# GATB/leon

Hardware: AMD Instinct MI355X
Metric: compressed input MB/s (DNA encode path) (higher is better)
Workload: dtype u64

## Files before the change

leon_amd/capi.py:

```python
import ctypes as C
import os

import numpy as np

_HERE = os.path.dirname(os.path.abspath(__file__))

ABI_VERSION = 5
HEADER_TEXT_DEVICE_CAP = 4096
LEON_F_KEEP_TRACE = 1
LEON_F_DICT_ON_DEVICE = 2


class LeonDnaError(RuntimeError):
    def __init__(self, code, msg):
        super().__init__("leon_dna error %d: %s" % (code, msg))
        self.code = code


def lib_path():
    return os.path.join(_HERE, "lib", "libleon_dna.so")


class _Cfg(C.Structure):
    _fields_ = [("struct_size", C.c_uint32), ("kmer_size", C.c_uint32), ("reads_per_block", C.c_uint32),
# ... 100 lines not shown
    "leon_device_count": (C.c_int, [C.POINTER(C.c_int)]),
    "leon_device_alloc": (C.c_int, [C.c_int, C.c_uint64, C.POINTER(C.c_void_p)]),
    "leon_device_upload": (C.c_int, [C.c_int, C.c_void_p, C.c_void_p, C.c_uint64]),
    "leon_device_copy": (C.c_int, [C.c_int, C.c_void_p, C.c_void_p, C.c_uint64]),
    "leon_device_download": (C.c_int, [C.c_int, C.c_void_p, C.c_void_p, C.c_uint64]),
    "leon_host_qual_encode_blocks": (C.c_int, [C.c_char_p, _u64p, C.c_uint64, C.c_uint32, C.c_int, C.c_uint32, SINK, C.c_void_p,
                                                C.c_uint64]),
    "leon_qual_deflate_blocks_device": (C.c_int, [C.c_int, C.c_void_p, _u64p, C.c_uint64, C.c_uint32, SINK, C.c_void_p, C.c_uint64]),
    "leon_qual_deflate_release": (None, []),
    "leon_device_trim": (None, []),
    "leon_host_qual_decode_blocks": (C.c_int, [_u8p, _u64p, _u32p, _u64p, C.c_uint64, _u8p, C.c_uint64, _u64p, C.c_uint32]),
    "leon_qual_inflate_blocks_device": (C.c_int, [C.c_int, C.c_void_p, C.c_void_p, C.c_void_p, C.c_void_p, C.c_uint64, C.c_void_p, C.c_void_p,
                                                   C.c_uint64, C.c_void_p, C.POINTER(C.c_uint64)]),
}
EXPORTED_SYMBOLS = tuple(_EXPORTS)
_lib = None


def load_library():
    global _lib
    if _lib is not None:
        return _lib
    path = lib_path()
    if not os.path.exists(path):
        raise LeonDnaError(-2, "%s is missing: build it with leon_amd.build_library() (hipcc, gfx950); "
                               "there is no CPU fallback" % path)
    lib = C.CDLL(path)
    for name, (res, args) in _EXPORTS.items():
        f = getattr(lib, name)
        f.restype, f.argtypes = res, args
    if lib.leon_dna_abi_version() != ABI_VERSION:
        raise LeonDnaError(-2, "%s has ABI %d, this binding is written for %d: rebuild it (leon_amd.build_library())"
                           % (path, lib.leon_dna_abi_version(), ABI_VERSION))
    _lib = lib
    return lib


def _ptr(a, t):
    return a.ctypes.data_as(t)


def kmer_words(k):
    return 2 if k >= 32 else 1


def anchor_dict_decode(payload, n_anchors, kmer_size):
    lib = load_library()
    out = np.zeros(max(n_anchors * kmer_words(kmer_size), 1), dtype=np.uint64)
    buf = np.frombuffer(bytes(payload) + b"\0", dtype=np.uint8)
    rc = lib.leon_host_anchor_dict_decode(_ptr(buf, _u8p), len(payload), n_anchors, kmer_size, _ptr(out, _u64p))
    if rc:
        raise LeonDnaError(rc, (lib.leon_last_error(None) or b"").decode())
    return out[:n_anchors * kmer_words(kmer_size)]


def host_anchor_dict_encode(kmers, k):
    lib = load_library()
    kmers = np.ascontiguousarray(kmers, dtype=np.uint64).reshape(-1)
    n = len(kmers) // kmer_words(k)
    cap = n * k + 64
    out = np.zeros(cap, dtype=np.uint8)
    size = C.c_uint64()
    rc = lib.leon_host_anchor_dict_encode(_ptr(kmers, _u64p), n, k, _ptr(out, _u8p), cap, C.byref(size))
    if rc:
        raise LeonDnaError(rc, "leon_host_anchor_dict_encode failed")
    return out[:size.value].tobytes()
# ... 565 lines not shown
                    self._xch_error = e
                    return 1
            self._gather_cb = GATHER(thunk)
        self._chk(self.lib.leon_dna_set_gather(self.h, self._gather_cb, None))

    def reset_stream(self):
        self._hdr_next = 0
        self._chk(self.lib.leon_dna_reset_stream(self.h))
        self.next_read = 0

    def stats(self):
        s = Stats()
        self._chk(self.lib.leon_dna_get_stats(self.h, C.byref(s)))
        return s.as_dict()

    def trace_anchors(self, n_reads):
        pos = np.zeros(n_reads, dtype=np.int32)
        addr = np.zeros(n_reads, dtype=np.uint32)
        flags = np.zeros(n_reads, dtype=np.uint8)
        self._chk(self.lib.leon_dna_trace_anchors(self.h, _ptr(pos, _i32p), _ptr(addr, _u32p), _ptr(flags, _u8p), n_reads))
        return pos, addr, flags

    def trace_events(self, n_bases):
        ev = np.zeros(n_bases, dtype=np.uint8)
        self._chk(self.lib.leon_dna_trace_events(self.h, _ptr(ev, _u8p), n_bases))
        return ev

    def anchor_kmers(self, n):
        w = kmer_words(self.kmer_size)
        out = np.zeros(max(n, 1) * w, dtype=np.uint64)
        self._chk(self.lib.leon_dna_anchor_kmers(self.h, _ptr(out, _u64p), n))
        return out[:n * w]

    def rc_encode_streams(self, syms, begin):
        syms = np.ascontiguousarray(syms, dtype=np.uint8)
        begin = np.ascontiguousarray(begin, dtype=np.uint64)
        ns = len(begin) - 1
        cap = 3 * (len(syms) // 2) + 64 * (ns + 1)
        out = np.zeros(cap, dtype=np.uint8)
        sizes = np.zeros(max(ns, 1), dtype=np.uint64)
        self._chk(self.lib.leon_rc_encode_streams(self.h, _ptr(syms, _u8p), _ptr(begin, _u64p), ns, _ptr(out, _u8p), cap,
                                                  _ptr(sizes, _u64p)))
        res, w = [], 0
        for i in range(ns):
            res.append(out[w:w + int(sizes[i])].tobytes())
            w += int(sizes[i])
        return res
```

leon_amd/csrc/capi.hip:

```cpp
#include "../../include/leon_dna.h"
#include "kernels.h"
#include "host_rc.h"
#include "staging.h"
#include "host_blocks.h"

#include "prim.h"

#include <algorithm>
#include <atomic>
#include <chrono>
#include <cstdio>
#include <cstdlib>
#include <cstring>
#include <functional>
#include <mutex>
#include <string>
#include <thread>
#include <vector>

using namespace leon;

namespace {

thread_local std::string g_create_error;
// ... 2164 lines not shown
int leon_dna_trace_events(leon_dna_ctx* c, uint8_t* events, uint64_t n_bases) {
    if (!c || !events) return LEON_E_INVALID;
    if (n_bases != c->last_bases) return fail(c, LEON_E_INVALID, "trace size differs from the last batch");
    HIPCHK(c, hipSetDevice(c->device));
    HIPCHK(c, hipMemcpy(events, c->events.p, n_bases, hipMemcpyDeviceToHost));
    return LEON_OK;
}
int leon_dna_anchor_kmers(leon_dna_ctx* c, uint64_t* kmers, uint64_t n) {
    if (!c || (!kmers && n)) return LEON_E_INVALID;
    if (n > c->n_anchors) return fail(c, LEON_E_INVALID, "more anchors requested than exist");
    HIPCHK(c, hipSetDevice(c->device));
    if (n) HIPCHK(c, hipMemcpy(kmers, c->anchor_kmers.p, n * 8 * kmer_words(c->cfg.kmer_size), hipMemcpyDeviceToHost));
    return LEON_OK;
}

int leon_host_anchor_dict_encode(const uint64_t* kmers, uint64_t n, uint32_t k, uint8_t* out, uint64_t out_cap, uint64_t* size) {
    if ((!kmers && n) || !size || k < 1 || k > 63) return LEON_E_INVALID;
    AnchorDictWorker worker(k);
    const uint32_t W = kmer_words(k);
    const uint64_t step = std::max<uint64_t>(1, n / 3);
    for (uint64_t i = 0; i < n; i += step) {
        const uint64_t m = std::min(step, n - i);
        worker.push(std::vector<uint64_t>(kmers + i * W, kmers + (i + m) * W));
    }
    worker.drain();
    AnchorDictCoder& coder = worker.coder();
    coder.flush();
    *size = coder.size();
    if (coder.size() > out_cap) return LEON_E_OVERFLOW;
    if (out) memcpy(out, coder.data(), coder.size());
    return LEON_OK;
}

int leon_rc_encode_streams(leon_dna_ctx* c, const uint8_t* syms, const uint64_t* begin, uint64_t n_streams,
                           uint8_t* out, uint64_t out_cap, uint64_t* sizes) {
    if (!c || !begin || !sizes || (!out && out_cap)) return LEON_E_INVALID;
    if (!n_streams) return LEON_OK;
    HIPCHK(c, hipSetDevice(c->device));
    hipStream_t s = c->stream;
    uint64_t n_syms = begin[n_streams] - begin[0];
    if (begin[0] != 0) return fail(c, LEON_E_INVALID, "begin[0] must be 0");
    for (uint64_t i = 0; i < n_syms; i++) {
        uint32_t m = syms[2 * i], v = syms[2 * i + 1];
        if (m >= N_MODELS || (m < N_SMALL_MODELS && v >= small_model_size(m))) return fail(c, LEON_E_INVALID, "bad symbol");
    }
    TmpBuf dsyms, dbegin, doff, dsize, dout, dscr;
    HIPCHK(c, dsyms.ensure(n_syms * 2 + 256)); HIPCHK(c, dbegin.ensure((n_streams + 1) * 8)); HIPCHK(c, doff.ensure((n_streams + 1) * 8));
    HIPCHK(c, dsize.ensure(n_streams * 8)); HIPCHK(c, dscr.ensure(rc_model_scratch_bytes(n_streams)));
    std::vector<uint64_t> off(n_streams + 1);
    for (uint64_t b = 0; b <= n_streams; b++) off[b] = ((3 * begin[b] + 7) & ~7ull) + 64 * b;
    HIPCHK(c, dout.ensure(off[n_streams] + 64));
    if (n_syms) HIPCHK(c, hipMemcpy(dsyms.p, syms, n_syms * 2, hipMemcpyHostToDevice));
    HIPCHK(c, hipMemcpy(dbegin.p, begin, (n_streams + 1) * 8, hipMemcpyHostToDevice));
    HIPCHK(c, hipMemcpy(doff.p, off.data(), (n_streams + 1) * 8, hipMemcpyHostToDevice));
    HIPCHK(c, hipMemsetAsync(c->errflag.p, 0, 4, s));
    uint64_t longest = 0;
    for (uint64_t b = 0; b < n_streams; b++) longest = std::max(longest, begin[b + 1] - begin[b]);
    if (const char* e = getenv("LEON_RC_STREAMS_ON_HOST")) if (e[0] == '1' && longest + 1024 < (1ull << HB_COUNT_BITS)) {
        if (int rc = rc_blocks_on_host(c, dsyms.as<uint8_t>(), dbegin.as<uint64_t>(), n_streams, n_syms, SMALL_SIZES_DNA, N_SMALL_MODELS))
            return rc == 1 ? fail(c, LEON_E_HIP, "no memory for the host chains' records") : rc;
        uint64_t w = 0;
        for (uint64_t b = 0; b < n_streams; b++) {
            sizes[b] = c->hb_coders[b].size();
            if (w + sizes[b] > out_cap) return fail(c, LEON_E_OVERFLOW, "out_cap too small");
            memcpy(out + w, c->hb_coders[b].data(), sizes[b]);
            w += sizes[b];
        }
        return LEON_OK;
    }
    launch_rc_encode(s, dsyms.as<uint8_t>(), dbegin.as<uint64_t>(), n_streams, dout.as<uint8_t>(), doff.as<uint64_t>(),
                     dsize.as<uint64_t>(), dscr.as<uint32_t>(), c->errflag.as<int>(), longest);
    HIPCHK(c, hipGetLastError());
    HIPCHK(c, hipStreamSynchronize(s));
    int errflag = 0;
    HIPCHK(c, hipMemcpy(&errflag, c->errflag.p, 4, hipMemcpyDeviceToHost));
    HIPCHK(c, hipMemcpy(sizes, dsize.p, n_streams * 8, hipMemcpyDeviceToHost));
    int rc = LEON_OK;
    if (errflag) rc = fail(c, LEON_E_OVERFLOW, "range coder output exceeded its bound");
    uint64_t w = 0;
    for (uint64_t b = 0; b < n_streams && rc == LEON_OK; b++) {
        if (w + sizes[b] > out_cap) { rc = fail(c, LEON_E_OVERFLOW, "out_cap too small"); break; }
        hipError_t e = hipMemcpy(out + w, dout.as<uint8_t>() + off[b], sizes[b], hipMemcpyDeviceToHost);
        if (e != hipSuccess) { rc = fail(c, LEON_E_HIP, hipGetErrorString(e)); break; }
        w += sizes[b];
    }
    return rc;
}

}
```

leon_amd/csrc/kernels.h:

```cpp
#pragma once
#include <hip/hip_runtime.h>
#include <stdint.h>
#include "leon_device.h"

namespace leon {

struct ReadsDev {
    const uint32_t* packed;
    const uint32_t* nmask;
    const uint64_t* slot_off;
    const uint64_t* base_off;
    const uint32_t* len;
    const uint32_t* n_count;
    uint64_t n;
    uint64_t ev_origin;
    uint32_t k, pad;
};

struct DictDev {
    uint64_t* slots;
    uint64_t* tent;
    uint64_t tstride;
    uint32_t* addr;
    uint64_t mask;
// ... 63 lines not shown
void launch_chain_prep(hipStream_t s, bool fill, ReadsDev R, DictDev D, ResolveDev V, uint64_t first_global, uint64_t w0, const uint32_t* list,
                       uint32_t n, uint32_t c0, const uint32_t* rank, uint32_t* cnt, uint32_t* own, const uint64_t* gbase, uint32_t* ent,
                       const unsigned long long* om, const unsigned long long* late, unsigned long long* dep, unsigned long long* xdep);
void launch_chain_tables(hipStream_t s, const uint32_t* cnt, const uint32_t* own, uint32_t n, uint64_t* rows ,
                         unsigned long long* om , unsigned long long* late );
int launch_chain_seq(hipStream_t s, uint32_t n, const uint32_t* cnt, const uint32_t* own, const unsigned long long* dep, const unsigned long long* xdep,
                     const uint64_t* gbase, const uint32_t* ent, unsigned long long* ins , unsigned long long* trace );
void launch_chain_apply(hipStream_t s, DictDev D, ResolveDev V, uint64_t first_global, const uint32_t* list, uint32_t n, const unsigned long long* ins, uint32_t k);
void launch_anchor_symbols(hipStream_t s, const uint64_t* kmers, uint64_t n_anchors, uint32_t k, uint8_t* syms);
void launch_finalize_reads(hipStream_t s, ReadsDev R, DictDev D, ResolveDev V, uint64_t w0, uint64_t w1);
struct WalkCache { uint64_t* slots; uint64_t bucket_mask; uint32_t hop_shift, pad; };
void launch_walk_cache_init(hipStream_t s, WalkCache C, uint32_t k);
void launch_walk(hipStream_t s, ReadsDev R, BloomDev B, const uint16_t* rv16, const int32_t* anchor_pos, const uint8_t* flags,
                 const uint32_t* perm, uint64_t n_walk, uint8_t* events, const uint64_t* ev_off = nullptr ,
                 WalkCache wc = WalkCache{nullptr, 0, 28, 0});
void launch_lower_bound(hipStream_t s, const uint64_t* sorted, uint64_t n, uint64_t bound, unsigned long long* out);
void launch_slice_weights(hipStream_t s, const uint64_t* sorted_keys, uint64_t n, uint64_t* w );
void launch_slice_splits(hipStream_t s, const uint64_t* cum , uint64_t n, uint32_t world, unsigned long long* split );
void launch_slice_reads(hipStream_t s, ReadsDev R, const uint32_t* perm , uint64_t n_slice, uint64_t* len_out ,
                        uint32_t* slot_of );
void launch_ev_words(hipStream_t s, ReadsDev R, const uint32_t* slot_of, const uint64_t* ev_off, const uint8_t* events, uint64_t n, uint32_t rpb,
                     uint64_t n_blocks, uint32_t world, uint64_t* cnt_or_off , uint64_t* send );
void launch_ev_scatter(hipStream_t s, const uint64_t* words, uint64_t n_words, uint8_t* events, uint64_t n_bytes, int* err);
void launch_prev_anchored(hipStream_t s, const int32_t* anchor_pos, uint64_t n, uint32_t rpb, uint64_t first_block,
                          uint64_t n_blocks, int64_t* prev);
void launch_symbols(hipStream_t s, ReadsDev R, const int32_t* anchor_pos, const uint32_t* anchor_addr,
                    const uint8_t* flags, const int64_t* prev, const uint8_t* events, uint64_t r0, uint64_t n_local,
                    uint64_t* sym_off , uint32_t* n_err ,
                    uint8_t* syms );
void launch_block_ranges(hipStream_t s, const uint64_t* sym_off, uint64_t n_reads, uint32_t rpb, uint64_t n_blocks,
                         uint64_t* blk_begin , uint64_t* out_off );
void launch_max_block_syms(hipStream_t s, const uint64_t* sym_off , uint64_t n_reads, uint32_t rpb, uint64_t n_blocks,
                           unsigned long long* out_max );
void launch_rc_encode(hipStream_t s, const uint8_t* syms, const uint64_t* blk_begin, uint64_t n_blocks,
                      uint8_t* out, const uint64_t* out_off, uint64_t* out_size, uint32_t* model_scratch, int* err,
                      uint64_t max_block_syms, uint32_t small_sizes = SMALL_SIZES_DNA, bool counts_apart = false);
size_t rc_records_state_bytes(uint64_t n_blocks);
void launch_rc_records(hipStream_t s, const uint8_t* syms, const uint64_t* blk_begin, uint64_t n_blocks, uint32_t tile0, uint32_t tile1, uint64_t* recs,
                       const uint64_t* rec_off, uint32_t* state, uint32_t* model_scratch, int* err, uint32_t small_sizes);
void launch_hdr_symbols(hipStream_t s, const uint8_t* hdr, const uint64_t* off, uint64_t n, uint32_t rpb, const uint8_t* first,
                        uint32_t first_len, uint64_t* sym_off , uint8_t* syms );
size_t rc_model_scratch_bytes(uint64_t n_blocks);
void launch_gather_payload(hipStream_t s, const uint8_t* out, const uint64_t* out_off, const uint64_t* dst_off,
                           const uint64_t* sizes, uint64_t n_blocks, uint8_t* dst);

void launch_qual_smooth(hipStream_t s, ReadsDev R, BloomDev B, const uint16_t* rv16, uint8_t* quals);
void launch_read_minimizer(hipStream_t s, ReadsDev R, uint32_t* key , uint32_t* mpos );
void launch_mpos_from_anchors(hipStream_t s, ReadsDev R, const int32_t* anchor_pos, const uint32_t* anchor_addr, const uint8_t* flags, uint32_t* key, uint32_t* mpos);
void launch_solid_flags(hipStream_t s, ReadsDev R, BloomDev B, const uint16_t* rv16, const uint32_t* perm, const uint32_t* mpos,
                        uint32_t* flags );
void launch_qual_rewrite(hipStream_t s, ReadsDev R, const uint32_t* flags, uint8_t* quals);
struct PathCache { uint64_t* slots; uint64_t bucket_mask; };
size_t path_cache_slot_bytes(uint32_t k);
void launch_path_cache_init(hipStream_t s, PathCache C, uint32_t k);
void launch_path_cache_prewalk(hipStream_t s, BloomDev B, PathCache C, const uint16_t* rv16, const uint64_t* anchors, uint64_t n_anchors, uint32_t max_steps);
void launch_bloom_fingerprint(hipStream_t s, const uint8_t* bits, uint64_t n_bytes, uint64_t* d_sum );
size_t decode_scratch_bytes(uint64_t n_blocks);
void launch_hdr_decode_symbols(hipStream_t s, const uint8_t* payloads, const uint64_t* pay_off, const uint32_t* blk_reads, uint64_t n_blocks,
                               uint8_t* syms, const uint64_t* sym_begin, unsigned long long* sym_count, int* err);
constexpr uint32_t LEON_HT_HEADER_CAP = 4096;
enum : uint32_t { HT_OK = 0, HT_LONG = 1, HT_SHARE = 2, HT_SYMS = 3, HT_NOSYMS = 4, HT_INVALID = 16 };
void launch_hdr_text(hipStream_t s, const uint8_t* syms, const uint64_t* sym_begin, const unsigned long long* sym_count, const uint32_t* blk_reads,
                     const uint64_t* read0, const uint64_t* text_begin, uint64_t n_blocks, const uint8_t* first, uint32_t first_len,
                     uint8_t* text , uint64_t* off, uint32_t* status, uint64_t* text_size);
void launch_decode_blocks(hipStream_t s, BloomDev B, PathCache C, const uint16_t* rv16, const uint64_t* anchors, uint64_t n_anchors,
                          const uint8_t* payloads, const uint64_t* pay_off, const uint32_t* blk_reads, const uint64_t* blk_read0,
                          const uint64_t* blk_out0, uint64_t n_blocks, uint8_t* out, uint32_t* out_len, uint32_t* scratch,
                          uint32_t* pool, unsigned long long* pool_cursor, uint64_t pool_words, int* err,
                          unsigned long long* stats );
// ... 31 lines not shown
```

leon_amd/csrc/rc_kernels.hip:

```cpp
#include "kernels.h"
#include "rc_model.h"
#include <algorithm>
#include <cstdlib>

namespace leon {

size_t rc_model_scratch_bytes(uint64_t n_blocks) {
    return (size_t)n_blocks * (RC_NNUM - RC_NSLOT_SMALL) * RC_STRIDE * sizeof(uint32_t);
}

__host__ __device__ constexpr uint32_t rc_waves(uint32_t g) { return g + 1 + (g - 1) / 3; }

__device__ inline void rc_rank_loop(uint32_t key, uint32_t c, uint32_t& lo, uint32_t& hi, uint32_t& tot) {
    const uint32_t lowkey = key & ~0xFFu;
    uint32_t sk0, sk1, dd;
    uint64_t m1, m2, sav;
    asm volatile(
        "s_mov_b64 %[sav], exec\n\t"
        "v_readlane_b32 %[sk0], %[key], 0\n\t"
        "s_mov_b64 exec, -2\n\t"
        "s_nop 1\n\t"
        ".set rc_i, 0\n\t"
        ".rept 32\n\t"
        "v_sub_u32 %[dd], %[sk0], %[lowkey]\n\t"
        "v_readlane_b32 %[sk1], %[key], rc_i + 1\n\t"
        "v_cmp_lt_u32 vcc, %[dd], %[c]\n\t"
        "v_cmp_le_u32 %[m1], %[dd], %[c]\n\t"
        "v_cmp_gt_u32 %[m2], %[k256], %[dd]\n\t"
        "v_addc_co_u32 %[lo], vcc, 0, %[lo], vcc\n\t"
        "v_addc_co_u32 %[hi], %[m1], 0, %[hi], %[m1]\n\t"
        "v_addc_co_u32 %[tot], %[m2], 0, %[tot], %[m2]\n\t"
        "s_lshl_b64 exec, exec, 1\n\t"
        "v_sub_u32 %[dd], %[sk1], %[lowkey]\n\t"
        "v_readlane_b32 %[sk0], %[key], (rc_i + 2) & 63\n\t"
// ... 88 lines not shown
        rc_rank_loop(key, c, lo, hi, tot);
        {
            if (!act) { lo = 0; hi = 1; tot = 1; }
        }
        {
            const bool in_lds = act && !(mb & RC_GLOBAL);
            uint32_t* mp = &models[in_lds ? mb : 0];
            const uint32_t h4 = (in_lds && numeric) ? c >> 4 : 64u;
            const uint32_t l4 = in_lds ? c & 15u : 64u, ymax = numeric ? 15u : (cmodel ? 16u : small_size_of(small_sizes, m));
            uint32_t* lp = mp + RC_LW + (in_lds ? (c & ~15u) : 0u);
#pragma unroll
            for (uint32_t k = 1; k <= 16; k++)
                if (k > h4) (void)__hip_atomic_fetch_add(&mp[k], 1u, __ATOMIC_RELAXED, __HIP_MEMORY_SCOPE_WAVEFRONT);
#pragma unroll
            for (uint32_t y = 1; y <= (CMP ? 16u : 15u); y++)
                if (y > l4 && y <= ymax) (void)__hip_atomic_fetch_add(&lp[y], 1u, __ATOMIC_RELAXED, __HIP_MEMORY_SCOPE_WAVEFRONT);
            unsigned long long gl = __ballot(act && (mb & RC_GLOBAL));
            while (gl) {
                const uint32_t i = (uint32_t)__builtin_ctzll(gl);
                gl &= gl - 1;
                const uint32_t ci = (uint32_t)__builtin_amdgcn_readlane((int)c, (int)i);
                const uint32_t mbi = (uint32_t)__builtin_amdgcn_readlane((int)mb, (int)i);
                const uint32_t thr = is_lw ? (ci & 15u) : (ci >> 4);
                const uint32_t idx = upd_base + ((ci & ~15u) & upd_blkmask);
                if (upd_lane > thr)
                    (void)__hip_atomic_fetch_add(gmodels + (mbi & ~RC_GLOBAL) + idx, 1u, __ATOMIC_RELAXED, __HIP_MEMORY_SCOPE_WAVEFRONT);
                asm volatile("s_waitcnt vmcnt(0)" ::: "memory");
            }
        }
        __builtin_amdgcn_wave_barrier();
    }
};

template <bool EXACT>
__device__ inline void rc_coder_tile(const uint4* ra, const uint2* rb, uint64_t& low, uint64_t& range, uint32_t& nout, uint8_t* dst, uint32_t cap) {
    uint4 pa = ra[0], pa1 = ra[1];
    uint2 pb = rb[0], pb1 = rb[1];
#pragma clang loop unroll_count(EXACT ? 1 : 4)
    for (uint32_t j = 0; j < 64; j++) {
        const uint32_t s_lo = pa.x, s_fr = pa.y, s_tot = pa.z, s_hc = pa.w, b0 = pb.x, b1 = pb.y;
        const uint32_t jn = j + 2 < 64 ? j + 2 : 64;
        pa = pa1; pb = pb1; pa1 = ra[jn]; pb1 = rb[jn];
        uint64_t top;
        if (EXACT) {
            const uint64_t q = range / (uint64_t)s_tot;
            const uint32_t q0 = (uint32_t)q, q1 = (uint32_t)(q >> 32);
            top = (uint64_t)q0 * s_hc + low;   top += (uint64_t)(q1 * s_hc) << 32;
            low = (uint64_t)q0 * s_lo + low;   low += (uint64_t)(q1 * s_lo) << 32;
            range = (uint64_t)q0 * s_fr;       range += (uint64_t)(q1 * s_fr) << 32;
        } else {
            const uint32_t r0 = (uint32_t)range, r1 = (uint32_t)(range >> 32);
            uint64_t qe = (uint64_t)r1 * b1 + __umulhi(r1, b0);
            qe += __umulhi(r0, b1);
            const uint32_t q0 = (uint32_t)qe, q1 = (uint32_t)(qe >> 32);
            uint64_t T0 = (uint64_t)q0 * s_hc + low;   T0 += (uint64_t)(q1 * s_hc) << 32;
            uint64_t L0 = (uint64_t)q0 * s_lo + low;   L0 += (uint64_t)(q1 * s_lo) << 32;
            uint64_t R0 = (uint64_t)q0 * s_fr;         R0 += (uint64_t)(q1 * s_fr) << 32;
            asm volatile("" : "+v"(T0), "+v"(L0), "+v"(R0));
            const uint32_t rem = r0 - q0 * s_tot;
            const uint32_t t2 = s_tot << 1, t3 = t2 + s_tot;
            uint32_t e = (rem >= s_tot ? 1u : 0u) + (rem >= t2 ? 1u : 0u) + (rem >= t3 ? 1u : 0u);
            asm volatile("" : "+v"(e));
            top = (uint64_t)e * s_hc + T0;
            low = (uint64_t)e * s_lo + L0;
            range = (uint64_t)e * s_fr + R0;
        }
        const uint32_t lh = (uint32_t)(low >> 32);
        uint32_t xh = lh ^ (uint32_t)(top >> 32);
        uint32_t lead;
        asm("v_ffbh_u32 %0, %1" : "=v"(lead), "+v"(xh));
        const uint32_t sh = lead & 24u;
        const uint64_t range_s = range << sh;
        uint32_t rare_below = xh == 0u ? 0xFFFFFFFFu : 0xFFFFu;
        asm volatile("" : "+v"(rare_below));
        const bool rare = (uint32_t)(range_s >> 32) <= rare_below;
        {
            const uint32_t cap4 = cap - 4;
            *(uint32_t*)(dst + (nout < cap4 ? nout : cap4)) = __builtin_bswap32(lh);
        }
        uint64_t low_n = low << sh, range_n = range_s;
        uint32_t nout_n = nout + (sh >> 3);
        if (__builtin_expect(__builtin_amdgcn_ballot_w64(rare) != 0, 0) && rare) {
            low_n = low; range_n = range; nout_n = nout;
            while ((low_n ^ (low_n + range_n)) < (1ull << 56) ||
                   (range_n < RC_BOTTOM && ((range_n = (0 - low_n) & (RC_BOTTOM - 1)), true))) {
                if (nout_n < cap) dst[nout_n] = (uint8_t)(low_n >> 56);
                nout_n++;
                range_n <<= 8;
                low_n <<= 8;
            }
        }
        low = low_n; range = range_n; nout = nout_n;
    }
}

template <uint32_t G, uint32_t RC_NSLOT, bool BIGOK, bool CMP>
__global__ void __launch_bounds__(64 * rc_waves(G)) k_rc_encode(const uint8_t* syms, const uint64_t* blk_begin, uint64_t n_blocks,
                                                            uint8_t* out, const uint64_t* out_off, uint64_t* out_size,
                                                            uint32_t* scratch, int* err, uint32_t small_sizes, uint32_t fast_total) {
    constexpr uint32_t MW = RcModeler<RC_NSLOT, CMP>::WORDS;
    __shared__ uint32_t models_all[G * MW];
    __shared__ uint4 ring_a[G][2][RC_RING];
    __shared__ uint2 ring_b[G][2][RC_RING];
    __shared__ uint8_t slotmap_all[G][RC_NNUM];
    __shared__ uint32_t ntiles_s[G];
    __shared__ uint32_t tile_big[BIGOK ? G : 1][2];
    const uint32_t lane = threadIdx.x & 63;
    const uint32_t wave = (uint32_t)__builtin_amdgcn_readfirstlane((int)(threadIdx.x >> 6));
    const bool is_coder = wave == 0, is_idle = wave != 0 && (wave & 3u) == 0;
    const uint32_t mi = is_coder || is_idle ? 0 : wave - 1 - (wave >> 2);
    RcModeler<RC_NSLOT, CMP> M;
    M.init(models_all + mi * MW, slotmap_all[mi], (const uint16_t*)syms, small_sizes, lane, err);

    const uint64_t n_groups = (n_blocks + G - 1) / G;
    for (uint64_t bg = blockIdx.x; bg < n_groups; bg += gridDim.x) {
        const uint64_t b = bg * G + (is_coder ? lane : mi);
        bool valid = (is_coder ? lane < G : !is_idle) && b < n_blocks;
        uint64_t s0 = 0, s1 = 0;
        if (valid) { s0 = blk_begin[b]; s1 = blk_begin[b + 1]; }
        if (valid && s1 - s0 >= 0xFFFFFF00ull) {
            if (is_coder || lane == 0) atomicExch(err, 2);
            if (is_coder) out_size[b] = 0;
            valid = false;
        }
        const uint32_t ntiles = valid ? (uint32_t)((s1 - s0 + 63) / 64) : 0;
        if (!is_coder && !is_idle && lane == 0) ntiles_s[mi] = ntiles;
        uint64_t low = 0, range = ~0ull;
        uint32_t nout = 0;
        uint8_t* dst = nullptr;
        uint32_t cap = 0;
        if (is_coder && valid) {
            dst = out + out_off[b];
            const uint64_t room = out_off[b + 1] - out_off[b];
            cap = (uint32_t)(room < 0xFFFFFFFFull ? room : 0xFFFFFFFFull);
        }
        if (!is_coder && !is_idle && valid)
            M.start_block(s0, s1, scratch + b * (uint64_t)(RC_NNUM - RC_NSLOT_SMALL) * RC_STRIDE, lane);
        __syncthreads();
        uint32_t T = 0;
        for (uint32_t w = 0; w < G; w++) T = ntiles_s[w] > T ? ntiles_s[w] : T;

        for (uint32_t t = 0; t <= T; t++) {
            if (is_idle) {
            } else if (!is_coder) {
                if (t < ntiles) {
                    uint32_t lo, hi, tot;
                    M.tile(t, lane, lo, hi, tot);
                    const uint64_t inv = ~0ull / (uint64_t)tot;
                    ring_a[mi][t & 1][lane] = make_uint4(lo, hi - lo, tot, hi);
                    ring_b[mi][t & 1][lane] = make_uint2((uint32_t)inv, (uint32_t)(inv >> 32));
                    if (BIGOK) {
                        const bool big = __ballot(tot >= fast_total) != 0;
                        if (lane == 0) tile_big[mi][t & 1] = big ? 1u : 0u;
                    }
                } else if (t < T) {
                    ring_a[mi][t & 1][lane] = make_uint4(0u, 1u, 1u, 1u);
                    ring_b[mi][t & 1][lane] = make_uint2(~0u, ~0u);
                    if (BIGOK && lane == 0) tile_big[mi][t & 1] = 0u;
                }
            } else if (t > 0) {
                if (valid) {
                    const uint4* ra = &ring_a[lane][(t - 1) & 1][0];
                    const uint2* rb = &ring_b[lane][(t - 1) & 1][0];
                    bool any_big = false;
                    if (BIGOK) any_big = __ballot(tile_big[lane < G ? lane : 0][(t - 1) & 1] != 0 && lane < G) != 0;
                    if (!BIGOK || __builtin_expect(!any_big, 1)) rc_coder_tile<false>(ra, rb, low, range, nout, dst, cap);
                    else rc_coder_tile<true>(ra, rb, low, range, nout, dst, cap);
                }
            }
            __syncthreads();
        }
        if (is_coder && valid) {
            for (int i = 0; i < 8; i++) {
                if (nout < cap) dst[nout] = (uint8_t)(low >> 56);
                nout++;
                low <<= 8;
            }
            out_size[b] = nout;
            if (nout > cap) atomicExch(err, 1);
        }
        __syncthreads();
    }
}

constexpr uint32_t RCR_MW = RC_SMALL_WORDS + RC_NSLOT_BIG * RC_STRIDE;
constexpr uint32_t RCR_STATE_WORDS = RCR_MW + RC_NNUM / 4 + 4;
size_t rc_records_state_bytes(uint64_t n_blocks) { return (size_t)n_blocks * RCR_STATE_WORDS * sizeof(uint32_t); }

__global__ void __launch_bounds__(64) k_rc_records(const uint8_t* syms, const uint64_t* blk_begin, uint64_t n_blocks, uint32_t tile0, uint32_t tile1,
                                                  uint64_t* recs, const uint64_t* rec_off, uint32_t* state, uint32_t* scratch, int* err, uint32_t small_sizes) {
    __shared__ uint32_t models[RCR_MW];
    __shared__ uint32_t slotmap_w[RC_NNUM / 4];
    uint8_t* slotmap = (uint8_t*)slotmap_w;
    const uint32_t lane = threadIdx.x;
    RcModeler<RC_NSLOT_BIG, false> M;
    M.init(models, slotmap, (const uint16_t*)syms, small_sizes, lane, err);
    for (uint64_t b = blockIdx.x; b < n_blocks; b += gridDim.x) {
        const uint64_t s0 = blk_begin[b], s1 = blk_begin[b + 1];
        if (s1 - s0 >= (1ull << 22) - 512) { if (lane == 0) atomicExch(err, 2); continue; }
        const uint32_t ntiles = (uint32_t)((s1 - s0 + 63) / 64);
        const uint32_t ta = tile0 < ntiles ? tile0 : ntiles, tb = tile1 < ntiles ? tile1 : ntiles;
        if (ta >= tb) continue;
        uint32_t* st = state + b * (uint64_t)RCR_STATE_WORDS;
        uint32_t* gm = scratch + b * (uint64_t)(RC_NNUM - RC_NSLOT_SMALL) * RC_STRIDE;
        if (ta == 0) M.start_block(s0, s1, gm, lane);
        else {
            for (uint32_t i = lane; i < RCR_MW; i += 64) models[i] = st[i];
            for (uint32_t i = lane; i < RC_NNUM / 4; i += 64) slotmap_w[i] = st[RCR_MW + i];
            M.s0 = s0; M.s1 = s1; M.gmodels = gm;
            M.nused = st[RCR_MW + RC_NNUM / 4];
            const uint64_t base = s0 + (uint64_t)ta * 64;
            M.raw_next = lane < (uint32_t)((s1 - base) < 64 ? (s1 - base) : 64) ? M.sym16[base + lane] : 0xFFFFu;
        }
        __syncthreads();
        uint64_t* out = recs + rec_off[b];
// ... 110 lines not shown
                while (gl) {
                    const uint32_t i = (uint32_t)__builtin_ctzll(gl);
                    gl &= gl - 1;
                    const uint32_t ci = (uint32_t)__builtin_amdgcn_readlane((int)c, (int)i);
                    const uint32_t mbi = (uint32_t)__builtin_amdgcn_readlane((int)mb, (int)i);
                    const uint32_t thr = is_lw ? (ci & 15u) : (ci >> 4);
                    const uint32_t idx = upd_base + ((ci & ~15u) & upd_blkmask);
                    if (upd_lane > thr) (void)__hip_atomic_fetch_add(gm + (mbi & ~RC_GLOBAL) + idx, 1u, __ATOMIC_RELAXED, __HIP_MEMORY_SCOPE_AGENT);
                    asm volatile("s_waitcnt vmcnt(0)" ::: "memory");
                }
            }
            asm volatile("s_waitcnt lgkmcnt(0)" ::: "memory");
            __atomic_signal_fence(__ATOMIC_SEQ_CST);
            __hip_atomic_store(&turn, t + 1, __ATOMIC_RELAXED, __HIP_MEMORY_SCOPE_WORKGROUP);
        }
        __syncthreads();
        if (tb < ntiles) {
            for (uint32_t i = threadIdx.x; i < RCR_MW; i += 256) st[i] = models[i];
            for (uint32_t i = threadIdx.x; i < RC_NNUM / 4; i += 256) st[RCR_MW + i] = slotmap_w[i];
            if (threadIdx.x == 0) st[RCR_MW + RC_NNUM / 4] = nused_s;
        }
    }
}
void launch_rc_records(hipStream_t s, const uint8_t* syms, const uint64_t* blk_begin, uint64_t n_blocks, uint32_t tile0, uint32_t tile1, uint64_t* recs,
                       const uint64_t* rec_off, uint32_t* state, uint32_t* model_scratch, int* err, uint32_t small_sizes) {
    if (!n_blocks || tile0 >= tile1) return;
    static const bool one_wave = [] { const char* e = getenv("LEON_RC_RECORDS_WAVES"); return e && atoi(e) == 1; }();
    if (one_wave) hipLaunchKernelGGL(k_rc_records, dim3((uint32_t)std::min<uint64_t>(n_blocks, 256 * 4)), dim3(64), 0, s, syms, blk_begin, n_blocks, tile0, tile1, recs, rec_off,
                                     state, model_scratch, err, small_sizes);
    else hipLaunchKernelGGL(k_rc_records4, dim3((uint32_t)std::min<uint64_t>(n_blocks, 256 * 4)), dim3(256), 0, s, syms, blk_begin, n_blocks, tile0, tile1, recs, rec_off,
                            state, model_scratch, err, small_sizes);
}

void launch_rc_encode(hipStream_t s, const uint8_t* syms, const uint64_t* blk_begin, uint64_t n_blocks, uint8_t* out,
                      const uint64_t* out_off, uint64_t* out_size, uint32_t* model_scratch, int* err, uint64_t max_block_syms, uint32_t small_sizes, bool counts_apart) {
    if (!n_blocks) return;
    const uint64_t per_cu = (n_blocks + 255) / 256;
    const char* force = getenv("LEON_RC_GROUP");
    uint32_t G = per_cu <= 1 ? 1u : per_cu <= 2 ? 2u : per_cu <= 4 ? 4u : 8u;
    if (force) { int v = atoi(force); if (v == 1 || v == 2 || v == 4 || v == 8) G = (uint32_t)v; }
    const uint64_t n_groups = (n_blocks + G - 1) / G;
    const uint32_t g = (uint32_t)std::min<uint64_t>(n_groups, 256ull * (8 / G));
    uint32_t fast_total = RC_MAX_TOTAL;
    if (const char* e = getenv("LEON_RC_FAST_TOTAL_LOG2")) { const int v = atoi(e); if (v >= 4 && v <= 30) fast_total = 1u << v; }
    const bool big = max_block_syms + 512 >= fast_total;
    const bool cmp = counts_apart && [] { const char* e = getenv("LEON_RC_CMP"); return !e || atoi(e) != 0; }();
#define RC_LAUNCH(GG, N, B, C) hipLaunchKernelGGL((k_rc_encode<GG, N, B, C>), dim3(g), dim3(64 * rc_waves(GG)), 0, s, syms, blk_begin, n_blocks, out, out_off, out_size, model_scratch, err, small_sizes, fast_total)
#define RC_PICK(GG, N, C) do { if (big) RC_LAUNCH(GG, N, true, C); else RC_LAUNCH(GG, N, false, C); } while (0)
    if (cmp) {
        if (G == 1) RC_PICK(1, RC_NSLOT_BIG, true);
        else if (G == 2) RC_PICK(2, RC_NSLOT_BIG, true);
        else if (G == 4) RC_PICK(4, RC_NSLOT_BIG, true);
        else RC_PICK(8, RC_NSLOT_SMALL, true);
    } else {
        if (G == 1) RC_PICK(1, RC_NSLOT_BIG, false);
        else if (G == 2) RC_PICK(2, RC_NSLOT_BIG, false);
        else if (G == 4) RC_PICK(4, RC_NSLOT_BIG, false);
        else RC_PICK(8, RC_NSLOT_SMALL + 1, false);
    }
#undef RC_PICK
#undef RC_LAUNCH
}

}
```

Baseline: 18720.

## Carry range-coder quotient forward via precomputed fixed-point ratios instead of per-symbol reciprocal division

Replaces the per-symbol quotient estimate, which used a stored 64-bit reciprocal of the total plus a correction step, with a recurrence. The next quotient range/total_next is derived from the current quotient times a precomputed ratio freq/total_next, split into an integer part A and a 64-bit fraction C. A full division runs only when the renormalisation is rare or the low bits leave the result in doubt, which is meant to cut the multiply and correction work on the common path. It also adds a traced kernel variant and a C API entry point that count which path each symbol takes. In exchange it adds a wide multiply and a doubt check per symbol, and the result depends on subtle rounding correctness.

Measured after the change: 18640. No clear change (-0.5%).

```diff
diff --git a/leon_amd/capi.py b/leon_amd/capi.py
--- a/leon_amd/capi.py
+++ b/leon_amd/capi.py
@@ -156,6 +156,8 @@
     if lib.leon_dna_abi_version() != ABI_VERSION:
         raise LeonDnaError(-2, "%s has ABI %d, this binding is written for %d: rebuild it (leon_amd.build_library())"
                            % (path, lib.leon_dna_abi_version(), ABI_VERSION))
+    lib.leon_rc_encode_streams_trace.restype = C.c_int
+    lib.leon_rc_encode_streams_trace.argtypes = [C.c_void_p, _u8p, _u64p, C.c_uint64, _u8p, C.c_uint64, _u64p, _u64p]
     _lib = lib
     return lib
 
@@ -787,17 +789,22 @@
         self._chk(self.lib.leon_dna_anchor_kmers(self.h, _ptr(out, _u64p), n))
         return out[:n * w]
 
-    def rc_encode_streams(self, syms, begin):
+    def rc_encode_streams(self, syms, begin, trace=False):
         syms = np.ascontiguousarray(syms, dtype=np.uint8)
         begin = np.ascontiguousarray(begin, dtype=np.uint64)
         ns = len(begin) - 1
         cap = 3 * (len(syms) // 2) + 64 * (ns + 1)
         out = np.zeros(cap, dtype=np.uint8)
         sizes = np.zeros(max(ns, 1), dtype=np.uint64)
-        self._chk(self.lib.leon_rc_encode_streams(self.h, _ptr(syms, _u8p), _ptr(begin, _u64p), ns, _ptr(out, _u8p), cap,
-                                                  _ptr(sizes, _u64p)))
+        counts = np.zeros(4, dtype=np.uint64)
+        if trace:
+            self._chk(self.lib.leon_rc_encode_streams_trace(self.h, _ptr(syms, _u8p), _ptr(begin, _u64p), ns, _ptr(out, _u8p), cap,
+                                                            _ptr(sizes, _u64p), _ptr(counts, _u64p)))
+        else:
+            self._chk(self.lib.leon_rc_encode_streams(self.h, _ptr(syms, _u8p), _ptr(begin, _u64p), ns, _ptr(out, _u8p), cap,
+                                                      _ptr(sizes, _u64p)))
         res, w = [], 0
         for i in range(ns):
             res.append(out[w:w + int(sizes[i])].tobytes())
             w += int(sizes[i])
-        return res
+        return (res, [int(x) for x in counts]) if trace else res
diff --git a/leon_amd/csrc/capi.hip b/leon_amd/csrc/capi.hip
--- a/leon_amd/csrc/capi.hip
+++ b/leon_amd/csrc/capi.hip
@@ -2220,9 +2220,16 @@
     return LEON_OK;
 }
 
+int leon_rc_encode_streams_trace(leon_dna_ctx* c, const uint8_t* syms, const uint64_t* begin, uint64_t n_streams,
+                                 uint8_t* out, uint64_t out_cap, uint64_t* sizes, uint64_t* counts);
 int leon_rc_encode_streams(leon_dna_ctx* c, const uint8_t* syms, const uint64_t* begin, uint64_t n_streams,
                            uint8_t* out, uint64_t out_cap, uint64_t* sizes) {
+    return leon_rc_encode_streams_trace(c, syms, begin, n_streams, out, out_cap, sizes, nullptr);
+}
+int leon_rc_encode_streams_trace(leon_dna_ctx* c, const uint8_t* syms, const uint64_t* begin, uint64_t n_streams,
+                                 uint8_t* out, uint64_t out_cap, uint64_t* sizes, uint64_t* counts) {
     if (!c || !begin || !sizes || (!out && out_cap)) return LEON_E_INVALID;
+    if (counts) counts[0] = counts[1] = counts[2] = counts[3] = 0;
     if (!n_streams) return LEON_OK;
     HIPCHK(c, hipSetDevice(c->device));
     hipStream_t s = c->stream;
@@ -2232,7 +2239,8 @@
         uint32_t m = syms[2 * i], v = syms[2 * i + 1];
         if (m >= N_MODELS || (m < N_SMALL_MODELS && v >= small_model_size(m))) return fail(c, LEON_E_INVALID, "bad symbol");
     }
-    TmpBuf dsyms, dbegin, doff, dsize, dout, dscr;
+    TmpBuf dsyms, dbegin, doff, dsize, dout, dscr, dtrace;
+    if (counts) { HIPCHK(c, dtrace.ensure(4 * 8)); HIPCHK(c, hipMemsetAsync(dtrace.p, 0, 4 * 8, s)); }
     HIPCHK(c, dsyms.ensure(n_syms * 2 + 256)); HIPCHK(c, dbegin.ensure((n_streams + 1) * 8)); HIPCHK(c, doff.ensure((n_streams + 1) * 8));
     HIPCHK(c, dsize.ensure(n_streams * 8)); HIPCHK(c, dscr.ensure(rc_model_scratch_bytes(n_streams)));
     std::vector<uint64_t> off(n_streams + 1);
@@ -2244,7 +2252,7 @@
     HIPCHK(c, hipMemsetAsync(c->errflag.p, 0, 4, s));
     uint64_t longest = 0;
     for (uint64_t b = 0; b < n_streams; b++) longest = std::max(longest, begin[b + 1] - begin[b]);
-    if (const char* e = getenv("LEON_RC_STREAMS_ON_HOST")) if (e[0] == '1' && longest + 1024 < (1ull << HB_COUNT_BITS)) {
+    if (const char* e = getenv("LEON_RC_STREAMS_ON_HOST")) if (!counts && e[0] == '1' && longest + 1024 < (1ull << HB_COUNT_BITS)) {
         if (int rc = rc_blocks_on_host(c, dsyms.as<uint8_t>(), dbegin.as<uint64_t>(), n_streams, n_syms, SMALL_SIZES_DNA, N_SMALL_MODELS))
             return rc == 1 ? fail(c, LEON_E_HIP, "no memory for the host chains' records") : rc;
         uint64_t w = 0;
@@ -2256,10 +2264,13 @@
         }
         return LEON_OK;
     }
-    launch_rc_encode(s, dsyms.as<uint8_t>(), dbegin.as<uint64_t>(), n_streams, dout.as<uint8_t>(), doff.as<uint64_t>(),
-                     dsize.as<uint64_t>(), dscr.as<uint32_t>(), c->errflag.as<int>(), longest);
+    if (!launch_rc_encode(s, dsyms.as<uint8_t>(), dbegin.as<uint64_t>(), n_streams, dout.as<uint8_t>(), doff.as<uint64_t>(),
+                          dsize.as<uint64_t>(), dscr.as<uint32_t>(), c->errflag.as<int>(), longest, SMALL_SIZES_DNA, false,
+                          counts ? dtrace.as<unsigned long long>() : nullptr))
+        return fail(c, LEON_E_INVALID, "no traced instantiation of the range coder for streams this long");
     HIPCHK(c, hipGetLastError());
     HIPCHK(c, hipStreamSynchronize(s));
+    if (counts) HIPCHK(c, hipMemcpy(counts, dtrace.p, 4 * 8, hipMemcpyDeviceToHost));
     int errflag = 0;
     HIPCHK(c, hipMemcpy(&errflag, c->errflag.p, 4, hipMemcpyDeviceToHost));
     HIPCHK(c, hipMemcpy(sizes, dsize.p, n_streams * 8, hipMemcpyDeviceToHost));
diff --git a/leon_amd/csrc/kernels.h b/leon_amd/csrc/kernels.h
--- a/leon_amd/csrc/kernels.h
+++ b/leon_amd/csrc/kernels.h
@@ -119,9 +119,10 @@
                          uint64_t* blk_begin , uint64_t* out_off );
 void launch_max_block_syms(hipStream_t s, const uint64_t* sym_off , uint64_t n_reads, uint32_t rpb, uint64_t n_blocks,
                            unsigned long long* out_max );
-void launch_rc_encode(hipStream_t s, const uint8_t* syms, const uint64_t* blk_begin, uint64_t n_blocks,
+bool launch_rc_encode(hipStream_t s, const uint8_t* syms, const uint64_t* blk_begin, uint64_t n_blocks,
                       uint8_t* out, const uint64_t* out_off, uint64_t* out_size, uint32_t* model_scratch, int* err,
-                      uint64_t max_block_syms, uint32_t small_sizes = SMALL_SIZES_DNA, bool counts_apart = false);
+                      uint64_t max_block_syms, uint32_t small_sizes = SMALL_SIZES_DNA, bool counts_apart = false,
+                      unsigned long long* trace = nullptr);
 size_t rc_records_state_bytes(uint64_t n_blocks);
 void launch_rc_records(hipStream_t s, const uint8_t* syms, const uint64_t* blk_begin, uint64_t n_blocks, uint32_t tile0, uint32_t tile1, uint64_t* recs,
                        const uint64_t* rec_off, uint32_t* state, uint32_t* model_scratch, int* err, uint32_t small_sizes);
diff --git a/leon_amd/csrc/rc_kernels.hip b/leon_amd/csrc/rc_kernels.hip
--- a/leon_amd/csrc/rc_kernels.hip
+++ b/leon_amd/csrc/rc_kernels.hip
@@ -1,5 +1,6 @@
 #include "kernels.h"
 #include "rc_model.h"
+#include "rc_quot.h"
 #include <algorithm>
 #include <cstdlib>
 
@@ -154,72 +155,99 @@
     }
 };
 
-template <bool EXACT>
-__device__ inline void rc_coder_tile(const uint4* ra, const uint2* rb, uint64_t& low, uint64_t& range, uint32_t& nout, uint8_t* dst, uint32_t cap) {
+__device__ inline uint32_t rc_renorm_usual(uint64_t low, uint64_t top, uint64_t range, uint32_t nout, uint8_t* dst, uint32_t cap, bool& rare) {
+    const uint32_t lh = (uint32_t)(low >> 32);
+    uint32_t xh = lh ^ (uint32_t)(top >> 32);
+    uint32_t lead;
+    asm("v_ffbh_u32 %0, %1" : "=v"(lead), "+v"(xh));
+    const uint32_t sh = lead & 24u;
+    uint32_t rare_below = xh == 0u ? 0xFFFFFFFFu : 0xFFFFu;
+    asm volatile("" : "+v"(rare_below));
+    rare = (uint32_t)((range << sh) >> 32) <= rare_below;
+    const uint32_t cap4 = cap - 4;
+    *(uint32_t*)(dst + (nout < cap4 ? nout : cap4)) = __builtin_bswap32(lh);
+    return sh;
+}
+__device__ inline void rc_renorm_loop(uint64_t& low, uint64_t& range, uint32_t& nout, uint8_t* dst, uint32_t cap) {
+    while ((low ^ (low + range)) < (1ull << 56) ||
+           (range < RC_BOTTOM && ((range = (0 - low) & (RC_BOTTOM - 1)), true))) {
+        if (nout < cap) dst[nout] = (uint8_t)(low >> 56);
+        nout++;
+        range <<= 8;
+        low <<= 8;
+    }
+}
+
+__device__ inline void rc_coder_tile_exact(const uint4* ra, uint64_t& low, uint64_t& range, uint32_t& nout, uint8_t* dst, uint32_t cap) {
     uint4 pa = ra[0], pa1 = ra[1];
-    uint2 pb = rb[0], pb1 = rb[1];
-#pragma clang loop unroll_count(EXACT ? 1 : 4)
+#pragma clang loop unroll_count(1)
     for (uint32_t j = 0; j < 64; j++) {
-        const uint32_t s_lo = pa.x, s_fr = pa.y, s_tot = pa.z, s_hc = pa.w, b0 = pb.x, b1 = pb.y;
+        const uint32_t s_lo = pa.x, s_fr = pa.y, s_tot = pa.z, s_hc = s_lo + s_fr;
         const uint32_t jn = j + 2 < 64 ? j + 2 : 64;
-        pa = pa1; pb = pb1; pa1 = ra[jn]; pb1 = rb[jn];
-        uint64_t top;
-        if (EXACT) {
-            const uint64_t q = range / (uint64_t)s_tot;
-            const uint32_t q0 = (uint32_t)q, q1 = (uint32_t)(q >> 32);
-            top = (uint64_t)q0 * s_hc + low;   top += (uint64_t)(q1 * s_hc) << 32;
-            low = (uint64_t)q0 * s_lo + low;   low += (uint64_t)(q1 * s_lo) << 32;
-            range = (uint64_t)q0 * s_fr;       range += (uint64_t)(q1 * s_fr) << 32;
-        } else {
-            const uint32_t r0 = (uint32_t)range, r1 = (uint32_t)(range >> 32);
-            uint64_t qe = (uint64_t)r1 * b1 + __umulhi(r1, b0);
-            qe += __umulhi(r0, b1);
-            const uint32_t q0 = (uint32_t)qe, q1 = (uint32_t)(qe >> 32);
-            uint64_t T0 = (uint64_t)q0 * s_hc + low;   T0 += (uint64_t)(q1 * s_hc) << 32;
-            uint64_t L0 = (uint64_t)q0 * s_lo + low;   L0 += (uint64_t)(q1 * s_lo) << 32;
-            uint64_t R0 = (uint64_t)q0 * s_fr;         R0 += (uint64_t)(q1 * s_fr) << 32;
-            asm volatile("" : "+v"(T0), "+v"(L0), "+v"(R0));
-            const uint32_t rem = r0 - q0 * s_tot;
-            const uint32_t t2 = s_tot << 1, t3 = t2 + s_tot;
-            uint32_t e = (rem >= s_tot ? 1u : 0u) + (rem >= t2 ? 1u : 0u) + (rem >= t3 ? 1u : 0u);
-            asm volatile("" : "+v"(e));
-            top = (uint64_t)e * s_hc + T0;
-            low = (uint64_t)e * s_lo + L0;
-            range = (uint64_t)e * s_fr + R0;
-        }
-        const uint32_t lh = (uint32_t)(low >> 32);
-        uint32_t xh = lh ^ (uint32_t)(top >> 32);
-        uint32_t lead;
-        asm("v_ffbh_u32 %0, %1" : "=v"(lead), "+v"(xh));
-        const uint32_t sh = lead & 24u;
-        const uint64_t range_s = range << sh;
-        uint32_t rare_below = xh == 0u ? 0xFFFFFFFFu : 0xFFFFu;
-        asm volatile("" : "+v"(rare_below));
-        const bool rare = (uint32_t)(range_s >> 32) <= rare_below;
-        {
-            const uint32_t cap4 = cap - 4;
-            *(uint32_t*)(dst + (nout < cap4 ? nout : cap4)) = __builtin_bswap32(lh);
-        }
-        uint64_t low_n = low << sh, range_n = range_s;
+        pa = pa1; pa1 = ra[jn];
+        const uint64_t q = range / (uint64_t)s_tot;
+        const uint64_t top = rc_quot_mul(q, s_hc, low);
+        low = rc_quot_mul(q, s_lo, low);
+        range = rc_quot_mul(q, s_fr, 0);
+        bool rare;
+        const uint32_t sh = rc_renorm_usual(low, top, range, nout, dst, cap, rare);
+        uint64_t low_n = low << sh, range_n = range << sh;
         uint32_t nout_n = nout + (sh >> 3);
         if (__builtin_expect(__builtin_amdgcn_ballot_w64(rare) != 0, 0) && rare) {
             low_n = low; range_n = range; nout_n = nout;
-            while ((low_n ^ (low_n + range_n)) < (1ull << 56) ||
-                   (range_n < RC_BOTTOM && ((range_n = (0 - low_n) & (RC_BOTTOM - 1)), true))) {
-                if (nout_n < cap) dst[nout_n] = (uint8_t)(low_n >> 56);
-                nout_n++;
-                range_n <<= 8;
-                low_n <<= 8;
-            }
+            rc_renorm_loop(low_n, range_n, nout_n, dst, cap);
         }
         low = low_n; range = range_n; nout = nout_n;
     }
 }
 
-template <uint32_t G, uint32_t RC_NSLOT, bool BIGOK, bool CMP>
+__device__ inline uint64_t rc_div_total(uint64_t range, uint32_t total) { return total == 1u ? range : range / (uint64_t)total; }
+
+template <bool TRACE>
+__device__ inline void rc_coder_tile_q(const uint4* ra, const uint2* rb, uint64_t& low, uint64_t& range, uint32_t& nout, uint8_t* dst, uint32_t cap,
+                                       uint32_t* cnt) {
+    uint4 pa = ra[0], pa1 = ra[1];
+    uint2 pb = rb[0], pb1 = rb[1];
+    uint64_t q = rc_div_total(range, pa.z);
+    if (TRACE) cnt[2]++;
+#pragma clang loop unroll_count(4)
+    for (uint32_t j = 0; j < 64; j++) {
+        const uint32_t s_lo = pa.x, s_fr = pa.y, s_A = pa.w, s_hc = s_lo + s_fr;
+        const uint64_t C = (uint64_t)pb.x | ((uint64_t)pb.y << 32);
+        const uint32_t jn = j + 2 < 64 ? j + 2 : 64;
+        pa = pa1; pb = pb1; pa1 = ra[jn]; pb1 = rb[jn];
+        const uint32_t tn = pa.z;
+        const uint64_t top = rc_quot_mul(q, s_hc, low);
+        low = rc_quot_mul(q, s_lo, low);
+        range = rc_quot_mul(q, s_fr, 0);
+        uint64_t Phi, Plo;
+        rc_quot_product(q, C, s_A, Phi, Plo);
+        bool rare, doubt;
+        const uint32_t sh = rc_renorm_usual(low, top, range, nout, dst, cap, rare);
+        uint64_t low_n = low << sh, range_n = range << sh;
+        uint32_t nout_n = nout + (sh >> 3);
+        uint64_t q_n = rc_quot_next(q, Phi, Plo, sh, doubt);
+        const bool slow = rare || doubt;
+        if (TRACE) {
+            const uint32_t path = rare ? 3u : doubt ? 1u : 0u;
+            for (uint32_t i = 0; i < 4; i++) cnt[i] += path == i ? 1u : 0u;
+        }
+        if (__builtin_expect(__builtin_amdgcn_ballot_w64(slow) != 0, 0) && slow) {
+            if (rare) {
+                low_n = low; range_n = range; nout_n = nout;
+                rc_renorm_loop(low_n, range_n, nout_n, dst, cap);
+            }
+            q_n = rc_div_total(range_n, tn);
+        }
+        low = low_n; range = range_n; nout = nout_n; q = q_n;
+    }
+}
+
+template <uint32_t G, uint32_t RC_NSLOT, bool BIGOK, bool CMP, bool TRACE = false>
 __global__ void __launch_bounds__(64 * rc_waves(G)) k_rc_encode(const uint8_t* syms, const uint64_t* blk_begin, uint64_t n_blocks,
                                                             uint8_t* out, const uint64_t* out_off, uint64_t* out_size,
-                                                            uint32_t* scratch, int* err, uint32_t small_sizes, uint32_t fast_total) {
+                                                            uint32_t* scratch, int* err, uint32_t small_sizes, uint32_t fast_total,
+                                                            unsigned long long* trace) {
     constexpr uint32_t MW = RcModeler<RC_NSLOT, CMP>::WORDS;
     __shared__ uint32_t models_all[G * MW];
     __shared__ uint4 ring_a[G][2][RC_RING];
@@ -233,6 +261,11 @@
     const uint32_t mi = is_coder || is_idle ? 0 : wave - 1 - (wave >> 2);
     RcModeler<RC_NSLOT, CMP> M;
     M.init(models_all + mi * MW, slotmap_all[mi], (const uint16_t*)syms, small_sizes, lane, err);
+    if (!is_coder && !is_idle && lane < 2) {
+        ring_a[mi][lane][RC_RING - 1] = make_uint4(0u, 1u, 1u, 0u);
+        ring_b[mi][lane][RC_RING - 1] = make_uint2(0u, 0u);
+    }
+    uint32_t cnt[4] = {0u, 0u, 0u, 0u};
 
     const uint64_t n_groups = (n_blocks + G - 1) / G;
     for (uint64_t bg = blockIdx.x; bg < n_groups; bg += gridDim.x) {
@@ -268,16 +301,18 @@
                 if (t < ntiles) {
                     uint32_t lo, hi, tot;
                     M.tile(t, lane, lo, hi, tot);
-                    const uint64_t inv = ~0ull / (uint64_t)tot;
-                    ring_a[mi][t & 1][lane] = make_uint4(lo, hi - lo, tot, hi);
-                    ring_b[mi][t & 1][lane] = make_uint2((uint32_t)inv, (uint32_t)(inv >> 32));
+                    const uint32_t tot_up = (uint32_t)__shfl_down((int)tot, 1);
+                    uint32_t A;
+                    const uint64_t C = rc_quot_c(hi - lo, lane < 63 ? tot_up : 0u, A);
+                    ring_a[mi][t & 1][lane] = make_uint4(lo, hi - lo, tot, A);
+                    ring_b[mi][t & 1][lane] = make_uint2((uint32_t)C, (uint32_t)(C >> 32));
                     if (BIGOK) {
                         const bool big = __ballot(tot >= fast_total) != 0;
                         if (lane == 0) tile_big[mi][t & 1] = big ? 1u : 0u;
                     }
                 } else if (t < T) {
-                    ring_a[mi][t & 1][lane] = make_uint4(0u, 1u, 1u, 1u);
-                    ring_b[mi][t & 1][lane] = make_uint2(~0u, ~0u);
+                    ring_a[mi][t & 1][lane] = make_uint4(0u, 1u, 1u, lane < 63 ? 1u : 0u);
+                    ring_b[mi][t & 1][lane] = make_uint2(0u, 0u);
                     if (BIGOK && lane == 0) tile_big[mi][t & 1] = 0u;
                 }
             } else if (t > 0) {
@@ -286,8 +321,8 @@
                     const uint2* rb = &ring_b[lane][(t - 1) & 1][0];
                     bool any_big = false;
                     if (BIGOK) any_big = __ballot(tile_big[lane < G ? lane : 0][(t - 1) & 1] != 0 && lane < G) != 0;
-                    if (!BIGOK || __builtin_expect(!any_big, 1)) rc_coder_tile<false>(ra, rb, low, range, nout, dst, cap);
-                    else rc_coder_tile<true>(ra, rb, low, range, nout, dst, cap);
+                    if (!BIGOK || __builtin_expect(!any_big, 1)) rc_coder_tile_q<TRACE>(ra, rb, low, range, nout, dst, cap, cnt);
+                    else rc_coder_tile_exact(ra, low, range, nout, dst, cap);
                 }
             }
             __syncthreads();
@@ -303,6 +338,8 @@
         }
         __syncthreads();
     }
+    if (TRACE && is_coder)
+        for (uint32_t i = 0; i < 4; i++) if (cnt[i]) atomicAdd(trace + i, (unsigned long long)cnt[i]);
 }
 
 constexpr uint32_t RCR_MW = RC_SMALL_WORDS + RC_NSLOT_BIG * RC_STRIDE;
@@ -479,9 +516,10 @@
                             state, model_scratch, err, small_sizes);
 }
 
-void launch_rc_encode(hipStream_t s, const uint8_t* syms, const uint64_t* blk_begin, uint64_t n_blocks, uint8_t* out,
-                      const uint64_t* out_off, uint64_t* out_size, uint32_t* model_scratch, int* err, uint64_t max_block_syms, uint32_t small_sizes, bool counts_apart) {
-    if (!n_blocks) return;
+bool launch_rc_encode(hipStream_t s, const uint8_t* syms, const uint64_t* blk_begin, uint64_t n_blocks, uint8_t* out,
+                      const uint64_t* out_off, uint64_t* out_size, uint32_t* model_scratch, int* err, uint64_t max_block_syms, uint32_t small_sizes, bool counts_apart,
+                      unsigned long long* trace) {
+    if (!n_blocks) return true;
     const uint64_t per_cu = (n_blocks + 255) / 256;
     const char* force = getenv("LEON_RC_GROUP");
     uint32_t G = per_cu <= 1 ? 1u : per_cu <= 2 ? 2u : per_cu <= 4 ? 4u : 8u;
@@ -492,7 +530,16 @@
     if (const char* e = getenv("LEON_RC_FAST_TOTAL_LOG2")) { const int v = atoi(e); if (v >= 4 && v <= 30) fast_total = 1u << v; }
     const bool big = max_block_syms + 512 >= fast_total;
     const bool cmp = counts_apart && [] { const char* e = getenv("LEON_RC_CMP"); return !e || atoi(e) != 0; }();
-#define RC_LAUNCH(GG, N, B, C) hipLaunchKernelGGL((k_rc_encode<GG, N, B, C>), dim3(g), dim3(64 * rc_waves(GG)), 0, s, syms, blk_begin, n_blocks, out, out_off, out_size, model_scratch, err, small_sizes, fast_total)
+#define RC_LAUNCH_T(GG, N, B, C, T) hipLaunchKernelGGL((k_rc_encode<GG, N, B, C, T>), dim3(g), dim3(64 * rc_waves(GG)), 0, s, syms, blk_begin, n_blocks, out, out_off, out_size, model_scratch, err, small_sizes, fast_total, trace)
+#define RC_LAUNCH(GG, N, B, C) RC_LAUNCH_T(GG, N, B, C, false)
+    if (trace) {
+        if (big || cmp) return false;
+        if (G == 1) RC_LAUNCH_T(1, RC_NSLOT_BIG, false, false, true);
+        else if (G == 2) RC_LAUNCH_T(2, RC_NSLOT_BIG, false, false, true);
+        else if (G == 4) RC_LAUNCH_T(4, RC_NSLOT_BIG, false, false, true);
+        else RC_LAUNCH_T(8, RC_NSLOT_SMALL + 1, false, false, true);
+        return true;
+    }
 #define RC_PICK(GG, N, C) do { if (big) RC_LAUNCH(GG, N, true, C); else RC_LAUNCH(GG, N, false, C); } while (0)
     if (cmp) {
         if (G == 1) RC_PICK(1, RC_NSLOT_BIG, true);
@@ -507,6 +554,8 @@
     }
 #undef RC_PICK
 #undef RC_LAUNCH
-}
-
-}
+#undef RC_LAUNCH_T
+    return true;
+}
+
+}
diff --git a/leon_amd/csrc/rc_quot.h b/leon_amd/csrc/rc_quot.h
--- /dev/null
+++ b/leon_amd/csrc/rc_quot.h
@@ -0,0 +1,68 @@
+#pragma once
+#include <cstdint>
+
+#if defined(__HIPCC__)
+#define RC_HD __host__ __device__
+#else
+#define RC_HD
+#endif
+#if defined(__HIP_DEVICE_COMPILE__)
+#define RC_OPAQUE32(x) asm volatile("" : "+v"(x))
+#else
+#define RC_OPAQUE32(x) (void)(x)
+#endif
+
+namespace leon {
+
+RC_HD inline uint32_t rc_quot_divstep(uint32_t hi, uint32_t d, double rd32, uint32_t& rem) {
+    uint64_t q = (uint64_t)((double)hi * rd32);
+    int64_t r = (int64_t)(((uint64_t)hi << 32) - q * d);
+    if (r < 0) { q--; r += d; }
+    else if (r >= (int64_t)d) { q++; r -= d; }
+    rem = (uint32_t)r;
+    return (uint32_t)q;
+}
+
+RC_HD inline uint64_t rc_quot_c(uint32_t freq, uint32_t total_next, uint32_t& A) {
+    if (!total_next) { A = 0; return 0ull; }
+    const double rd32 = 4294967296.0 / (double)total_next;
+    uint64_t a = (uint64_t)((double)freq * (rd32 * (1.0 / 4294967296.0)));
+    int64_t f = (int64_t)freq - (int64_t)(a * total_next);
+    if (f < 0) { a--; f += total_next; }
+    else if (f >= (int64_t)total_next) { a++; f -= total_next; }
+    A = (uint32_t)a;
+    uint32_t r;
+    const uint32_t hi = rc_quot_divstep((uint32_t)f, total_next, rd32, r);
+    const uint32_t lo = rc_quot_divstep(r, total_next, rd32, r);
+    return ((uint64_t)hi << 32) | lo;
+}
+
+RC_HD inline uint64_t rc_mad(uint32_t a, uint32_t b, uint64_t c) { return (uint64_t)a * b + c; }
+
+RC_HD inline uint64_t rc_quot_mul(uint64_t q, uint32_t x, uint64_t add) {
+    const uint32_t q0 = (uint32_t)q, q1 = (uint32_t)(q >> 32);
+    return rc_mad(q0, x, add) + ((uint64_t)(q1 * x) << 32);
+}
+
+RC_HD inline void rc_quot_product(uint64_t q, uint64_t C, uint32_t A, uint64_t& Phi, uint64_t& Plo) {
+    const uint32_t q0 = (uint32_t)q, q1 = (uint32_t)(q >> 32), c0 = (uint32_t)C, c1 = (uint32_t)(C >> 32);
+    const uint64_t t0 = rc_mad(q0, c0, 0);
+    const uint64_t t1 = rc_mad(q0, c1, t0 >> 32);
+    const uint64_t b = rc_mad(q1, c0, 0);
+    const uint64_t qa = rc_quot_mul(q, A, 0);
+    const uint64_t d = rc_mad(q1, c1, t1 >> 32);
+    const uint64_t u = b + (uint32_t)t1;
+    Phi = d + ((u >> 32) + qa);
+    Plo = (u << 32) | (uint32_t)t0;
+}
+
+RC_HD inline uint64_t rc_quot_next(uint64_t q, uint64_t Phi, uint64_t Plo, uint32_t sh, bool& doubt) {
+    const uint32_t in = (uint32_t)(((Plo >> 32) << sh) >> 32);
+    uint32_t hq = (uint32_t)((q << sh) >> 32), hp = (uint32_t)((~Plo << sh) >> 32);
+    RC_OPAQUE32(hq);
+    RC_OPAQUE32(hp);
+    doubt = hq >= hp;
+    return (Phi << sh) | in;
+}
+
+}
```
